# LeeBY68/Hier-SLAM

Hardware: AMD Instinct MI355X
Metric: fwd+bwd renders/sec @1200x680, 500k Gaussians, 4-level tree; grad max-abs-err vs ref (higher is better)
Workload: dtype f32; 1 GPU; semantic fwd+bwd render, 1200x680, P=500000 slam Gaussians, K=26 semantic channels, dense upstream grads on colour/semantic/depth/median/opacity; P=500000, visible=480888, num_rendered=1136056, width=1200, height=680, K=26, parallelism=single GPU, keyframes_per_rank=1

## Files before the change

### hier-slam_amd/csrc/hsr_sort.hip

```cpp
#include "hsr_common.h"

namespace {

constexpr int SORT_THREADS = 256;
constexpr int SORT_ITEMS = 16;
constexpr int SORT_TILE = SORT_THREADS * SORT_ITEMS;
static_assert(SORT_TILE == HSR_SORT_TILE, "hsr_common.h sizes the histogram scratch");

__global__ void __launch_bounds__(SORT_THREADS) sort_hist_kernel(const uint64_t* __restrict__ keys, int n, int shift,
                                                                 uint32_t mask, int nblocks, uint32_t* __restrict__ hist)
{
    __shared__ uint32_t h[256];
    h[threadIdx.x] = 0;
    __syncthreads();
    const int base = blockIdx.x * SORT_TILE;
#pragma unroll 4
    for (int i = 0; i < SORT_ITEMS; i++) {
        const int j = base + i * SORT_THREADS + threadIdx.x;
        if (j < n) atomicAdd(&h[(uint32_t)(keys[j] >> shift) & mask], 1u);
    }
    __syncthreads();
    hist[(size_t)threadIdx.x * nblocks + blockIdx.x] = h[threadIdx.x];
}

__global__ void __launch_bounds__(64) sort_rowscan_kernel(uint32_t* __restrict__ hist, int nblocks,
                                                           uint32_t* __restrict__ totals)
{
    const int lane = threadIdx.x;
    uint32_t* row = hist + (size_t)blockIdx.x * nblocks;
    uint32_t carry = 0;
    for (int base = 0; base < nblocks; base += 64) {
        const int j = base + lane;
        const uint32_t v = j < nblocks ? row[j] : 0u;
        uint32_t inc = v;
#pragma unroll
        for (int o = 1; o < 64; o <<= 1) {
            const uint32_t t = __shfl_up(inc, o);
            if (lane >= o) inc += t;
        }
        if (j < nblocks) row[j] = carry + inc - v;
        carry += __shfl(inc, 63);
    }
    if (lane == 0) totals[blockIdx.x] = carry;
}

__global__ void __launch_bounds__(SORT_THREADS) sort_scatter_kernel(const uint64_t* __restrict__ kin,
                                                                    const uint32_t* __restrict__ vin,
                                                                    uint64_t* __restrict__ kout, uint32_t* __restrict__ vout,
                                                                    int n, int shift, uint32_t mask, int nblocks,
                                                                    const uint32_t* __restrict__ hist_scanned,
                                                                    const uint32_t* __restrict__ totals)
{
    __shared__ uint32_t wcnt[4][256];
    __shared__ uint32_t dig_base[256];
    __shared__ uint32_t wtot[4];
    const int lane = threadIdx.x & 63, w = threadIdx.x >> 6;
#pragma unroll
    for (int i = 0; i < 4; i++) wcnt[i][threadIdx.x] = 0;
    __syncthreads();

    const int base = blockIdx.x * SORT_TILE + w * (64 * SORT_ITEMS);
    uint64_t key[SORT_ITEMS];
    uint32_t val[SORT_ITEMS];
    uint32_t rank[SORT_ITEMS];
    const uint64_t lt_mask = (1ull << lane) - 1ull;
    volatile uint32_t* mycnt = wcnt[w];
#pragma unroll
    for (int r = 0; r < SORT_ITEMS; r++) {
        const int j = base + r * 64 + lane;
        const bool valid = j < n;
        key[r] = valid ? kin[j] : 0ull;
        val[r] = valid ? vin[j] : 0u;
    }
#pragma unroll
    for (int r = 0; r < SORT_ITEMS; r++) {
        const int j = base + r * 64 + lane;
        const bool valid = j < n;
        const uint32_t d = (uint32_t)(key[r] >> shift) & mask;
        uint64_t m = __ballot(valid);
#pragma unroll
        for (int b = 0; b < 8; b++) {
            const bool bit = (d >> b) & 1u;
            const uint64_t bal = __ballot(bit);
            m &= bit ? bal : ~bal;
        }
        const uint32_t before = __popcll(m & lt_mask);
        const uint32_t prior = valid ? mycnt[d] : 0u;
        __builtin_amdgcn_wave_barrier();
        if (valid && before == 0) mycnt[d] = prior + (uint32_t)__popcll(m);
        __builtin_amdgcn_wave_barrier();
        rank[r] = prior + before;
    }
    {
        const uint32_t tv = totals[threadIdx.x];
        uint32_t inc = tv;
#pragma unroll
        for (int o = 1; o < 64; o <<= 1) {
            const uint32_t t = __shfl_up(inc, o);
            if (lane >= o) inc += t;
        }
        if (lane == 63) wtot[w] = inc;
        __syncthreads();
        uint32_t woff = 0;
#pragma unroll
        for (int i = 0; i < 4; i++) woff += i < w ? wtot[i] : 0u;
        dig_base[threadIdx.x] = woff + inc - tv;
    }
    {
        const uint32_t c0 = wcnt[0][threadIdx.x], c1 = wcnt[1][threadIdx.x], c2 = wcnt[2][threadIdx.x];
        const uint32_t g = dig_base[threadIdx.x] + hist_scanned[(size_t)threadIdx.x * nblocks + blockIdx.x];
        wcnt[0][threadIdx.x] = g;
        wcnt[1][threadIdx.x] = g + c0;
        wcnt[2][threadIdx.x] = g + c0 + c1;
        wcnt[3][threadIdx.x] = g + c0 + c1 + c2;
    }
    __syncthreads();
#pragma unroll
    for (int r = 0; r < SORT_ITEMS; r++) {
        const int j = base + r * 64 + lane;
        if (j < n) {
            const uint32_t d = (uint32_t)(key[r] >> shift) & mask;
            const uint32_t pos = wcnt[w][d] + rank[r];
            kout[pos] = key[r];
            vout[pos] = val[r];
        }
    }
}

}


constexpr int TS_MAX = 2048;

__device__ __forceinline__ void ts_block_radix(uint64_t* ka, uint32_t* va, uint64_t* kb, uint32_t* vb, int r0, int n,
                                               uint32_t* hist , uint32_t (*wcnt)[256], int gid_passes)
{
    const int t = threadIdx.x, lane = t & 63, w = t >> 6;
    const uint64_t lt = (1ull << lane) - 1ull;
    const int npass = gid_passes + 4;
    for (int pass = 0; pass < npass; pass++) {
        const bool on_gid = pass < gid_passes;
        const int shift = 8 * (on_gid ? pass : pass - gid_passes);
        hist[t] = 0;
#pragma unroll
        for (int i = 0; i < 4; i++) wcnt[i][t] = 0;
        __syncthreads();
        for (int i = t; i < n; i += 256)
            atomicAdd(&hist[((on_gid ? va[r0 + i] : (uint32_t)ka[r0 + i]) >> shift) & 255u], 1u);
        __syncthreads();
        {
            const uint32_t v = hist[t];
            uint32_t inc = v;
#pragma unroll
            for (int o = 1; o < 64; o <<= 1) {
                const uint32_t x = __shfl_up(inc, o);
                if (lane >= o) inc += x;
            }
            __shared__ uint32_t wt[4];
            if (lane == 63) wt[w] = inc;
            __syncthreads();
            uint32_t off = 0;
#pragma unroll
            for (int i = 0; i < 4; i++) off += i < w ? wt[i] : 0u;
            hist[t] = off + inc - v;
        }
        __syncthreads();
        for (int c = 0; c < n; c += 256) {
            const int i = c + t;
            const bool valid = i < n;
            const uint64_t k = valid ? ka[r0 + i] : 0ull;
            const uint32_t v = valid ? va[r0 + i] : 0u;
            const uint32_t d = ((on_gid ? v : (uint32_t)k) >> shift) & 255u;
            uint64_t m = __ballot(valid);
#pragma unroll
            for (int b = 0; b < 8; b++) {
                const bool bit = (d >> b) & 1u;
                const uint64_t bal = __ballot(bit);
                m &= bit ? bal : ~bal;
            }
            const uint32_t before = __popcll(m & lt);
            if (valid && before == 0) wcnt[w][d] = (uint32_t)__popcll(m);
            __syncthreads();
            if (valid) {
                uint32_t pos = hist[d] + before;
#pragma unroll
                for (int i2 = 0; i2 < 4; i2++) pos += i2 < w ? wcnt[i2][d] : 0u;
                kb[r0 + pos] = k;
                vb[r0 + pos] = v;
            }
            __syncthreads();
            hist[t] += wcnt[0][t] + wcnt[1][t] + wcnt[2][t] + wcnt[3][t];
#pragma unroll
            for (int i2 = 0; i2 < 4; i2++) wcnt[i2][t] = 0;
            __syncthreads();
        }
        uint64_t* tk = ka; ka = kb; kb = tk;
        uint32_t* tv = va; va = vb; vb = tv;
        __threadfence_block();
    }
    if (npass & 1) {
        __syncthreads();
        for (int i = t; i < n; i += 256) {
            kb[r0 + i] = ka[r0 + i];
            vb[r0 + i] = va[r0 + i];
        }
    }
}

constexpr int TP_MAX = 1024;
constexpr int TQ_MAX = 2048;

template <int E, int NT>
__device__ __forceinline__ void net_bitonic(uint64_t (&x)[E], int tid, ulonglong2* buf)
{
    constexpr int N = NT * E;
#pragma unroll
    for (int k = 2; k <= N; k <<= 1) {
#pragma unroll
        for (int j = k >> 1; j > 0; j >>= 1) {
            if (j < E) {
#pragma unroll
                for (int r = 0; r < E; r++) {
                    if ((r & j) == 0) {
                        const bool up = k < E ? ((r & k) == 0) : (((E * tid) & k) == 0);
                        const uint64_t a = x[r], b = x[r + j];
                        const bool sw = (a > b) == up;
                        x[r] = sw ? b : a;
                        x[r + j] = sw ? a : b;
                    }
                }
            } else {
                const int m = j / E;
                const bool cross = m >= 64;
#pragma unroll
                for (int q = 0; q < E / 2; q++) buf[q * NT + tid] = make_ulonglong2(x[2 * q], x[2 * q + 1]);
                if (cross) {
                    __syncthreads();
                } else {
                    __builtin_amdgcn_fence(__ATOMIC_RELEASE, "wavefront");
                    __builtin_amdgcn_wave_barrier();
                    __builtin_amdgcn_fence(__ATOMIC_ACQUIRE, "wavefront");
                }
                const bool keep_min = ((tid & m) == 0) == (((E * tid) & k) == 0);
#pragma unroll
                for (int q = 0; q < E / 2; q++) {
                    const ulonglong2 y = buf[q * NT + (tid ^ m)];
                    const uint64_t a0 = x[2 * q], a1 = x[2 * q + 1];
                    x[2 * q] = keep_min ? (a0 < y.x ? a0 : y.x) : (a0 > y.x ? a0 : y.x);
                    x[2 * q + 1] = keep_min ? (a1 < y.y ? a1 : y.y) : (a1 > y.y ? a1 : y.y);
                }
                if (cross) {
                    __syncthreads();
                } else {
                    __builtin_amdgcn_fence(__ATOMIC_RELEASE, "wavefront");
                    __builtin_amdgcn_wave_barrier();
                    __builtin_amdgcn_fence(__ATOMIC_ACQUIRE, "wavefront");
                }
            }
        }
    }
}

__device__ __forceinline__ void block_sort_tile(int tile, const uint2* __restrict__ ranges, uint64_t* __restrict__ keys,
                                                uint32_t* __restrict__ vals, uint64_t* __restrict__ keys_alt,
                                                uint32_t* __restrict__ vals_alt, int gid_passes, int composite_in, uint64_t* comp,
                                                uint32_t* hist, uint32_t (*wcnt)[256])
{
    const uint2 rg = ranges[tile];
    const int r0 = (int)rg.x, n = (int)(rg.y - rg.x);
    const int t = threadIdx.x;
    const uint64_t my_tile_hi = (uint64_t)tile << 32;
    if (n <= 0) return;
    if (n == 1 || n > TS_MAX) {
        if (composite_in) {
            for (int i = t; i < n; i += 256) {
                const uint64_t c = keys[r0 + i];
                keys[r0 + i] = my_tile_hi | (c >> 32);
                vals[r0 + i] = (uint32_t)c;
            }
            __syncthreads();
        }
        if (n == 1) return;
    }
    if (n > TS_MAX) {
        ts_block_radix(keys, vals, keys_alt, vals_alt, r0, n, hist, wcnt, gid_passes);
        return;
    }
    if (composite_in) {
        static_assert(TQ_MAX == TS_MAX && TS_MAX * 8 >= 4 * 256 * 16, "exchange buffer = the LDS network's key array");
        uint64_t x[8];
#pragma unroll
        for (int r = 0; r < 8; r++) {
            const int e = 8 * t + r;
            x[r] = e < n ? keys[r0 + e] : ~0ull;
        }
        net_bitonic<8, 256>(x, t, reinterpret_cast<ulonglong2*>(comp));
#pragma unroll
        for (int r = 0; r < 8; r++) {
            const int e = 8 * t + r;
            if (e < n) {
                keys[r0 + e] = my_tile_hi | (x[r] >> 32);
                vals[r0 + e] = (uint32_t)x[r];
            }
        }
        return;
    }
    int N = 64;
    while (N < n) N <<= 1;
    const uint64_t tile_hi = keys[r0] & 0xFFFFFFFF00000000ull;
    for (int i = t; i < N; i += 256)
        comp[i] = i < n ? (((keys[r0 + i] & 0xFFFFFFFFull) << 32) | (uint64_t)vals[r0 + i]) : ~0ull;
    __syncthreads();
    bool cross = false;
    for (int k = 2; k <= N; k <<= 1) {
        for (int j = k >> 1; j > 0; j >>= 1) {
            if (j >= 128 || cross) __syncthreads();
            cross = j >= 128;
            for (int i = t; i < N / 2; i += 256) {
                const int lo = ((i & ~(j - 1)) << 1) | (i & (j - 1));
                const int hi = lo | j;
                const bool up = (lo & k) == 0;
                const uint64_t a = comp[lo], b = comp[hi];
                if ((a > b) == up) {
                    comp[lo] = b;
                    comp[hi] = a;
                }
            }
        }
    }
    __syncthreads();
    for (int i = t; i < n; i += 256) {
        const uint64_t c = comp[i];
        keys[r0 + i] = tile_hi | (c >> 32);
        vals[r0 + i] = (uint32_t)c;
    }
}

__global__ void __launch_bounds__(256) tile_sort_kernel(const uint2* __restrict__ ranges, uint64_t* __restrict__ keys,
                                                        uint32_t* __restrict__ vals, uint64_t* __restrict__ keys_alt,
                                                        uint32_t* __restrict__ vals_alt, int gid_passes, int composite_in, BinDevRef ref)
{
    if (ref.base) {
        BinState bs;
        if (!hsr_bin_resolve(ref, *ref.R_dev, &bs)) return;
        keys = bs.keys; vals = bs.vals; keys_alt = bs.keys_unsorted; vals_alt = bs.vals_unsorted;
    }
    __shared__ uint64_t comp[TS_MAX];
    __shared__ uint32_t hist[256];
    __shared__ uint32_t wcnt[4][256];
    if (composite_in == 2) {
        const uint2 rg = ranges[blockIdx.x];
        if (rg.y - rg.x <= (uint32_t)TP_MAX) return;
        composite_in = 1;
    }
    block_sort_tile((int)blockIdx.x, ranges, keys, vals, keys_alt, vals_alt, gid_passes, composite_in, comp, hist, wcnt);
}

template <int E>
__device__ __forceinline__ void pair_sort_tile(int r0, int n, int tid, uint64_t tile_hi, uint64_t* __restrict__ keys,
                                               uint32_t* __restrict__ vals, ulonglong2* buf)
{
    uint64_t x[E];
#pragma unroll
    for (int r = 0; r < E; r++) {
        const int e = E * tid + r;
        x[r] = e < n ? keys[r0 + e] : ~0ull;
    }
    net_bitonic<E, 128>(x, tid, buf);
#pragma unroll
    for (int r = 0; r < E; r++) {
        const int e = E * tid + r;
        if (e < n) {
            keys[r0 + e] = tile_hi | (x[r] >> 32);
            vals[r0 + e] = (uint32_t)x[r];
        }
    }
}

__global__ void __launch_bounds__(256, 7) tile_sort_pair_kernel(int T, const uint2* __restrict__ ranges, uint64_t* __restrict__ keys,
                                                             uint32_t* __restrict__ vals, uint64_t* __restrict__ keys_alt,
                                                             uint32_t* __restrict__ vals_alt, int gid_passes, int big_too, BinDevRef ref)
{
    constexpr int RAW_WG = TS_MAX * 8 + 256 * 4 + 4 * 256 * 4, RAW_PAIR = 2 * 4 * 128 * 16;
    constexpr int RAW = RAW_WG > RAW_PAIR ? RAW_WG : RAW_PAIR;
    __shared__ __attribute__((aligned(16))) unsigned char s_raw[RAW];
    __shared__ int s_big[2];
    if (ref.base) {
        BinState bs;
        if (!hsr_bin_resolve(ref, *ref.R_dev, &bs)) return;
        keys = bs.keys; vals = bs.vals; keys_alt = bs.keys_unsorted; vals_alt = bs.vals_unsorted;
    }
    const int pair = threadIdx.x >> 7, tid = threadIdx.x & 127;
    const int tile = blockIdx.x * 2 + pair;
    int n = 0, r0 = 0;
    if (tile < T) {
        const uint2 rg = ranges[tile];
        r0 = (int)rg.x;
        n = (int)(rg.y - rg.x);
    }
    if (tid == 0) s_big[pair] = n > TP_MAX;
    {
        ulonglong2* buf = reinterpret_cast<ulonglong2*>(s_raw) + pair * (4 * 128);
        const uint64_t tile_hi = (uint64_t)tile << 32;
        if (n > 0 && n <= 256) pair_sort_tile<2>(r0, n, tid, tile_hi, keys, vals, buf);
        else if (n > 256 && n <= 512) pair_sort_tile<4>(r0, n, tid, tile_hi, keys, vals, buf);
        else if (n > 512 && n <= TP_MAX) pair_sort_tile<8>(r0, n, tid, tile_hi, keys, vals, buf);
        else { __syncthreads(); __syncthreads(); }
    }
    if (!big_too) return;
    __syncthreads();
    uint64_t* comp = reinterpret_cast<uint64_t*>(s_raw);
    uint32_t* hist = reinterpret_cast<uint32_t*>(s_raw + TS_MAX * 8);
    uint32_t (*wcnt)[256] = reinterpret_cast<uint32_t (*)[256]>(s_raw + TS_MAX * 8 + 256 * 4);
    for (int w = 0; w < 2; w++) {
        if (!s_big[w]) continue;
        block_sort_tile(blockIdx.x * 2 + w, ranges, keys, vals, keys_alt, vals_alt, gid_passes, 1, comp, hist, wcnt);
        __syncthreads();
    }
}

int hsr_sort_tile_passes(int end_bit)
{
    const int tile_bits = end_bit - 32;
    return tile_bits <= 0 ? 0 : (tile_bits + 7) / 8;
}
bool hsr_sort_emit_into_sorted_buffers(int end_bit) { return (hsr_sort_tile_passes(end_bit) & 1) == 0; }

int hsr_launch_sort_pairs(BinState& b, int R, int end_bit, int T, uint2* ranges, hipStream_t stream)
{
    if (R <= 0) return HSR_OK;
    const int passes = hsr_sort_tile_passes(end_bit);
    const int tile_bits = end_bit - 32;
    const int nblocks = (R + SORT_TILE - 1) / SORT_TILE;
    uint32_t* totals = b.hist + (size_t)256 * nblocks;
    uint64_t* ka = (passes & 1) ? b.keys_unsorted : b.keys;
    uint32_t* va = (passes & 1) ? b.vals_unsorted : b.vals;
    uint64_t* kb = (passes & 1) ? b.keys : b.keys_unsorted;
    uint32_t* vb = (passes & 1) ? b.vals : b.vals_unsorted;
    const int bits_per_pass = passes ? (tile_bits + passes - 1) / passes : 0;
    for (int p = 0; p < passes; p++) {
        const int shift = 32 + bits_per_pass * p;
        const int bits = min(bits_per_pass, end_bit - shift);
        const uint32_t mask = (1u << bits) - 1u;
        sort_hist_kernel<<<nblocks, SORT_THREADS, 0, stream>>>(ka, R, shift, mask, nblocks, b.hist);
        sort_rowscan_kernel<<<256, 64, 0, stream>>>(b.hist, nblocks, totals);
        sort_scatter_kernel<<<nblocks, SORT_THREADS, 0, stream>>>(ka, va, kb, vb, R, shift, mask, nblocks, b.hist, totals);
        uint64_t* tk = ka; ka = kb; kb = tk;
        uint32_t* tv = va; va = vb; vb = tv;
    }
    hsr_launch_tile_ranges_only(R, b.keys, ranges, stream);
    tile_sort_kernel<<<T, 256, 0, stream>>>(ranges, b.keys, b.vals, b.keys_unsorted, b.vals_unsorted, 0, 0, BinDevRef{nullptr, nullptr, 0});
    return HSR_OK;
}

int hsr_launch_tile_sort(BinState& b, int T, int P, const uint2* ranges, hipStream_t stream, const BinDevRef* ref, int avg_per_tile_hint)
{
    int bits = 0;
    while (bits < 32 && (1ull << bits) < (unsigned long long)(P > 1 ? P : 1)) bits++;
    const BinDevRef r = ref ? *ref : BinDevRef{nullptr, nullptr, 0};
    const bool many_big = avg_per_tile_hint > 800;
    tile_sort_pair_kernel<<<(T + 1) / 2, 256, 0, stream>>>(T, ranges, b.keys, b.vals, b.keys_unsorted, b.vals_unsorted, (bits + 7) / 8,
                                                           many_big ? 0 : 1, r);
    if (many_big)
        tile_sort_kernel<<<T, 256, 0, stream>>>(ranges, b.keys, b.vals, b.keys_unsorted, b.vals_unsorted, (bits + 7) / 8, 2, r);
    return HSR_OK;
}
```

Before: 1883 renders/s.

## Use ds_swizzle/permlane exchanges in bitonic tile sort and vectorize global I/O

The per-tile bitonic network now exchanges partners inside a wavefront using ds_swizzle and permlane32_swap register shuffles instead of writing to and reading back from LDS with wave barriers. Loads and stores of keys and values use 16-byte vector accesses when the segment is aligned. Pointers are also marked as global address space so the compiler can emit global rather than flat instructions. This is meant to cut LDS traffic and memory-instruction count in the tile sort stage, at the cost of two 32-bit shuffles per 64-bit element and more code complexity.

```diff
diff --git a/hier-slam_amd/csrc/hsr_sort.hip b/hier-slam_amd/csrc/hsr_sort.hip
--- a/hier-slam_amd/csrc/hsr_sort.hip
+++ b/hier-slam_amd/csrc/hsr_sort.hip
@@ -1,4 +1,5 @@
 #include "hsr_common.h"
+#include "hsr_sort_net.h"
 
 namespace {
 
@@ -132,7 +133,7 @@
 
 constexpr int TS_MAX = 2048;
 
-__device__ __forceinline__ void ts_block_radix(uint64_t* ka, uint32_t* va, uint64_t* kb, uint32_t* vb, int r0, int n,
+__device__ __forceinline__ void ts_block_radix(sg_u64* ka, sg_u32* va, sg_u64* kb, sg_u32* vb, int r0, int n,
                                                uint32_t* hist , uint32_t (*wcnt)[256], int gid_passes)
 {
     const int t = threadIdx.x, lane = t & 63, w = t >> 6;
@@ -194,8 +195,8 @@
             for (int i2 = 0; i2 < 4; i2++) wcnt[i2][t] = 0;
             __syncthreads();
         }
-        uint64_t* tk = ka; ka = kb; kb = tk;
-        uint32_t* tv = va; va = vb; vb = tv;
+        sg_u64* tk = ka; ka = kb; kb = tk;
+        sg_u32* tv = va; va = vb; vb = tv;
         __threadfence_block();
     }
     if (npass & 1) {
@@ -209,64 +210,14 @@
 
 constexpr int TP_MAX = 1024;
 constexpr int TQ_MAX = 2048;
-
-template <int E, int NT>
-__device__ __forceinline__ void net_bitonic(uint64_t (&x)[E], int tid, ulonglong2* buf)
-{
-    constexpr int N = NT * E;
-#pragma unroll
-    for (int k = 2; k <= N; k <<= 1) {
-#pragma unroll
-        for (int j = k >> 1; j > 0; j >>= 1) {
-            if (j < E) {
-#pragma unroll
-                for (int r = 0; r < E; r++) {
-                    if ((r & j) == 0) {
-                        const bool up = k < E ? ((r & k) == 0) : (((E * tid) & k) == 0);
-                        const uint64_t a = x[r], b = x[r + j];
-                        const bool sw = (a > b) == up;
-                        x[r] = sw ? b : a;
-                        x[r + j] = sw ? a : b;
-                    }
-                }
-            } else {
-                const int m = j / E;
-                const bool cross = m >= 64;
-#pragma unroll
-                for (int q = 0; q < E / 2; q++) buf[q * NT + tid] = make_ulonglong2(x[2 * q], x[2 * q + 1]);
-                if (cross) {
-                    __syncthreads();
-                } else {
-                    __builtin_amdgcn_fence(__ATOMIC_RELEASE, "wavefront");
-                    __builtin_amdgcn_wave_barrier();
-                    __builtin_amdgcn_fence(__ATOMIC_ACQUIRE, "wavefront");
-                }
-                const bool keep_min = ((tid & m) == 0) == (((E * tid) & k) == 0);
-#pragma unroll
-                for (int q = 0; q < E / 2; q++) {
-                    const ulonglong2 y = buf[q * NT + (tid ^ m)];
-                    const uint64_t a0 = x[2 * q], a1 = x[2 * q + 1];
-                    x[2 * q] = keep_min ? (a0 < y.x ? a0 : y.x) : (a0 > y.x ? a0 : y.x);
-                    x[2 * q + 1] = keep_min ? (a1 < y.y ? a1 : y.y) : (a1 > y.y ? a1 : y.y);
-                }
-                if (cross) {
-                    __syncthreads();
-                } else {
-                    __builtin_amdgcn_fence(__ATOMIC_RELEASE, "wavefront");
-                    __builtin_amdgcn_wave_barrier();
-                    __builtin_amdgcn_fence(__ATOMIC_ACQUIRE, "wavefront");
-                }
-            }
-        }
-    }
-}
-
-__device__ __forceinline__ void block_sort_tile(int tile, const uint2* __restrict__ ranges, uint64_t* __restrict__ keys,
-                                                uint32_t* __restrict__ vals, uint64_t* __restrict__ keys_alt,
-                                                uint32_t* __restrict__ vals_alt, int gid_passes, int composite_in, uint64_t* comp,
+constexpr int TS_XCH = SN_SWIZZLE;
+
+__device__ __forceinline__ void block_sort_tile(int tile, const sg_u32x2* __restrict__ ranges, sg_u64* __restrict__ keys,
+                                                sg_u32* __restrict__ vals, sg_u64* __restrict__ keys_alt,
+                                                sg_u32* __restrict__ vals_alt, int gid_passes, int composite_in, uint64_t* comp,
                                                 uint32_t* hist, uint32_t (*wcnt)[256])
 {
-    const uint2 rg = ranges[tile];
+    const sn_u32x2 rg = ranges[tile];
     const int r0 = (int)rg.x, n = (int)(rg.y - rg.x);
     const int t = threadIdx.x;
     const uint64_t my_tile_hi = (uint64_t)tile << 32;
@@ -288,21 +239,12 @@
     }
     if (composite_in) {
         static_assert(TQ_MAX == TS_MAX && TS_MAX * 8 >= 4 * 256 * 16, "exchange buffer = the LDS network's key array");
+        int tq = t;
+        asm volatile("" : "+v"(tq));
         uint64_t x[8];
-#pragma unroll
-        for (int r = 0; r < 8; r++) {
-            const int e = 8 * t + r;
-            x[r] = e < n ? keys[r0 + e] : ~0ull;
-        }
-        net_bitonic<8, 256>(x, t, reinterpret_cast<ulonglong2*>(comp));
-#pragma unroll
-        for (int r = 0; r < 8; r++) {
-            const int e = 8 * t + r;
-            if (e < n) {
-                keys[r0 + e] = my_tile_hi | (x[r] >> 32);
-                vals[r0 + e] = (uint32_t)x[r];
-            }
-        }
+        sn_load_run<8>(keys + r0, (r0 & 1) == 0, 8 * tq, n, x);
+        net_bitonic<8, 256, TS_XCH>(x, tq, reinterpret_cast<ulonglong2*>(comp));
+        sn_store_run<8>(keys + r0, vals + r0, r0, 8 * tq, n, my_tile_hi, x);
         return;
     }
     int N = 64;
@@ -345,36 +287,27 @@
         if (!hsr_bin_resolve(ref, *ref.R_dev, &bs)) return;
         keys = bs.keys; vals = bs.vals; keys_alt = bs.keys_unsorted; vals_alt = bs.vals_unsorted;
     }
+    const sg_u32x2* const ranges_g = (const sg_u32x2*)ranges;
     __shared__ uint64_t comp[TS_MAX];
     __shared__ uint32_t hist[256];
     __shared__ uint32_t wcnt[4][256];
     if (composite_in == 2) {
-        const uint2 rg = ranges[blockIdx.x];
+        const sn_u32x2 rg = ranges_g[blockIdx.x];
         if (rg.y - rg.x <= (uint32_t)TP_MAX) return;
         composite_in = 1;
     }
-    block_sort_tile((int)blockIdx.x, ranges, keys, vals, keys_alt, vals_alt, gid_passes, composite_in, comp, hist, wcnt);
+    block_sort_tile((int)blockIdx.x, ranges_g, (sg_u64*)keys, (sg_u32*)vals, (sg_u64*)keys_alt, (sg_u32*)vals_alt, gid_passes, composite_in,
+                    comp, hist, wcnt);
 }
 
 template <int E>
-__device__ __forceinline__ void pair_sort_tile(int r0, int n, int tid, uint64_t tile_hi, uint64_t* __restrict__ keys,
-                                               uint32_t* __restrict__ vals, ulonglong2* buf)
+__device__ __forceinline__ void pair_sort_tile(int r0, int n, int tid, uint64_t tile_hi, sg_u64* __restrict__ keys,
+                                               sg_u32* __restrict__ vals, ulonglong2* buf)
 {
     uint64_t x[E];
-#pragma unroll
-    for (int r = 0; r < E; r++) {
-        const int e = E * tid + r;
-        x[r] = e < n ? keys[r0 + e] : ~0ull;
-    }
-    net_bitonic<E, 128>(x, tid, buf);
-#pragma unroll
-    for (int r = 0; r < E; r++) {
-        const int e = E * tid + r;
-        if (e < n) {
-            keys[r0 + e] = tile_hi | (x[r] >> 32);
-            vals[r0 + e] = (uint32_t)x[r];
-        }
-    }
+    sn_load_run<E>(keys + r0, (r0 & 1) == 0, E * tid, n, x);
+    net_bitonic<E, 128, TS_XCH>(x, tid, buf);
+    sn_store_run<E>(keys + r0, vals + r0, r0, E * tid, n, tile_hi, x);
 }
 
 __global__ void __launch_bounds__(256, 7) tile_sort_pair_kernel(int T, const uint2* __restrict__ ranges, uint64_t* __restrict__ keys,
@@ -390,11 +323,14 @@
         if (!hsr_bin_resolve(ref, *ref.R_dev, &bs)) return;
         keys = bs.keys; vals = bs.vals; keys_alt = bs.keys_unsorted; vals_alt = bs.vals_unsorted;
     }
+    const sg_u32x2* const ranges_g = (const sg_u32x2*)ranges;
+    sg_u64* const keys_g = (sg_u64*)keys;
+    sg_u32* const vals_g = (sg_u32*)vals;
     const int pair = threadIdx.x >> 7, tid = threadIdx.x & 127;
     const int tile = blockIdx.x * 2 + pair;
     int n = 0, r0 = 0;
     if (tile < T) {
-        const uint2 rg = ranges[tile];
+        const sn_u32x2 rg = ranges_g[tile];
         r0 = (int)rg.x;
         n = (int)(rg.y - rg.x);
     }
@@ -402,9 +338,9 @@
     {
         ulonglong2* buf = reinterpret_cast<ulonglong2*>(s_raw) + pair * (4 * 128);
         const uint64_t tile_hi = (uint64_t)tile << 32;
-        if (n > 0 && n <= 256) pair_sort_tile<2>(r0, n, tid, tile_hi, keys, vals, buf);
-        else if (n > 256 && n <= 512) pair_sort_tile<4>(r0, n, tid, tile_hi, keys, vals, buf);
-        else if (n > 512 && n <= TP_MAX) pair_sort_tile<8>(r0, n, tid, tile_hi, keys, vals, buf);
+        if (n > 0 && n <= 256) pair_sort_tile<2>(r0, n, tid, tile_hi, keys_g, vals_g, buf);
+        else if (n > 256 && n <= 512) pair_sort_tile<4>(r0, n, tid, tile_hi, keys_g, vals_g, buf);
+        else if (n > 512 && n <= TP_MAX) pair_sort_tile<8>(r0, n, tid, tile_hi, keys_g, vals_g, buf);
         else { __syncthreads(); __syncthreads(); }
     }
     if (!big_too) return;
@@ -414,7 +350,7 @@
     uint32_t (*wcnt)[256] = reinterpret_cast<uint32_t (*)[256]>(s_raw + TS_MAX * 8 + 256 * 4);
     for (int w = 0; w < 2; w++) {
         if (!s_big[w]) continue;
-        block_sort_tile(blockIdx.x * 2 + w, ranges, keys, vals, keys_alt, vals_alt, gid_passes, 1, comp, hist, wcnt);
+        block_sort_tile(blockIdx.x * 2 + w, ranges_g, keys_g, vals_g, (sg_u64*)keys_alt, (sg_u32*)vals_alt, gid_passes, 1, comp, hist, wcnt);
         __syncthreads();
     }
 }
diff --git a/hier-slam_amd/csrc/hsr_sort_net.h b/hier-slam_amd/csrc/hsr_sort_net.h
--- /dev/null
+++ b/hier-slam_amd/csrc/hsr_sort_net.h
@@ -0,0 +1,185 @@
+#pragma once
+#include <hip/hip_runtime.h>
+#include <stdint.h>
+
+typedef __attribute__((address_space(1))) uint64_t sg_u64;
+typedef __attribute__((address_space(1))) uint32_t sg_u32;
+typedef uint64_t sn_u64x2 __attribute__((ext_vector_type(2)));
+typedef uint32_t sn_u32x2 __attribute__((ext_vector_type(2)));
+typedef uint32_t sn_u32x4 __attribute__((ext_vector_type(4)));
+typedef __attribute__((address_space(1))) sn_u64x2 sg_u64x2;
+typedef __attribute__((address_space(1))) sn_u32x2 sg_u32x2;
+typedef __attribute__((address_space(1))) sn_u32x4 sg_u32x4;
+
+enum { SN_LDS = 0, SN_BPERMUTE = 1, SN_SWIZZLE = 2, SN_DPP = 3, SN_MIX = 4 };
+
+template <int CTRL>
+__device__ __forceinline__ uint32_t sn_dpp(uint32_t v)
+{
+    return (uint32_t)__builtin_amdgcn_update_dpp(0, (int)v, CTRL, 0xf, 0xf, true);
+}
+
+template <int M>
+__device__ __forceinline__ uint32_t sn_swizzle_xor(uint32_t v)
+{
+    return (uint32_t)__builtin_amdgcn_ds_swizzle((int)v, 0x1f | (M << 10));
+}
+
+template <int XCH>
+__device__ __forceinline__ uint32_t sn_partner_dword(uint32_t v, int m, int lane)
+{
+    if (XCH == SN_BPERMUTE) return (uint32_t)__shfl_xor((int)v, m);
+    constexpr int QP_1032 = 0xB1, QP_2301 = 0x4E, QP_3210 = 0x1B, ROW_MIRROR = 0x140, ROW_HALF_MIRROR = 0x141;
+    if (XCH == SN_DPP || XCH == SN_MIX) {
+        switch (m) {
+        case 1: return sn_dpp<QP_1032>(v);
+        case 2: return sn_dpp<QP_2301>(v);
+        default: break;
+        }
+    }
+    if (XCH == SN_DPP) {
+        switch (m) {
+        case 4: return sn_dpp<QP_3210>(sn_dpp<ROW_HALF_MIRROR>(v));
+        case 8: return sn_dpp<ROW_HALF_MIRROR>(sn_dpp<ROW_MIRROR>(v));
+        case 16: {
+            const auto r = __builtin_amdgcn_permlane16_swap(v, v, false, false);
+            return (lane & 16) ? r[0] : r[1];
+        }
+        default: break;
+        }
+    }
+    switch (m) {
+    case 1: return sn_swizzle_xor<1>(v);
+    case 2: return sn_swizzle_xor<2>(v);
+    case 4: return sn_swizzle_xor<4>(v);
+    case 8: return sn_swizzle_xor<8>(v);
+    case 16: return sn_swizzle_xor<16>(v);
+    default: {
+        const auto r = __builtin_amdgcn_permlane32_swap(v, v, false, false);
+        return lane < 32 ? r[1] : r[0];
+    }
+    }
+}
+
+template <int E, int NT, int XCH = SN_LDS>
+__device__ __forceinline__ void net_bitonic(uint64_t (&x)[E], int tid, ulonglong2* buf)
+{
+    constexpr int N = NT * E;
+#pragma unroll
+    for (int k = 2; k <= N; k <<= 1) {
+#pragma unroll
+        for (int j = k >> 1; j > 0; j >>= 1) {
+            if (j < E) {
+#pragma unroll
+                for (int r = 0; r < E; r++) {
+                    if ((r & j) == 0) {
+                        const bool up = k < E ? ((r & k) == 0) : (((E * tid) & k) == 0);
+                        const uint64_t a = x[r], b = x[r + j];
+                        const bool sw = (a > b) == up;
+                        x[r] = sw ? b : a;
+                        x[r + j] = sw ? a : b;
+                    }
+                }
+            } else {
+                const int m = j / E;
+                const bool cross = m >= 64;
+                const bool keep_min = ((tid & m) == 0) == (((E * tid) & k) == 0);
+                if (cross || XCH == SN_LDS) {
+#pragma unroll
+                    for (int q = 0; q < E / 2; q++) buf[q * NT + tid] = make_ulonglong2(x[2 * q], x[2 * q + 1]);
+                    if (cross) {
+                        __syncthreads();
+                    } else {
+                        __builtin_amdgcn_fence(__ATOMIC_RELEASE, "wavefront");
+                        __builtin_amdgcn_wave_barrier();
+                        __builtin_amdgcn_fence(__ATOMIC_ACQUIRE, "wavefront");
+                    }
+#pragma unroll
+                    for (int q = 0; q < E / 2; q++) {
+                        const ulonglong2 y = buf[q * NT + (tid ^ m)];
+                        const uint64_t a0 = x[2 * q], a1 = x[2 * q + 1];
+                        x[2 * q] = ((a0 < y.x) == keep_min) ? a0 : y.x;
+                        x[2 * q + 1] = ((a1 < y.y) == keep_min) ? a1 : y.y;
+                    }
+                    if (cross) {
+                        __syncthreads();
+                    } else {
+                        __builtin_amdgcn_fence(__ATOMIC_RELEASE, "wavefront");
+                        __builtin_amdgcn_wave_barrier();
+                        __builtin_amdgcn_fence(__ATOMIC_ACQUIRE, "wavefront");
+                    }
+                } else {
+#pragma unroll
+                    for (int r = 0; r < E; r++) {
+                        const uint64_t a = x[r];
+                        const uint32_t ylo = sn_partner_dword<XCH>((uint32_t)a, m, tid & 63);
+                        const uint32_t yhi = sn_partner_dword<XCH>((uint32_t)(a >> 32), m, tid & 63);
+                        const uint64_t y = ((uint64_t)yhi << 32) | ylo;
+                        x[r] = ((a < y) == keep_min) ? a : y;
+                    }
+                }
+            }
+        }
+    }
+}
+
+template <int E>
+__device__ __forceinline__ void sn_load_run(const sg_u64* seg, bool seg_even, int e0, int n, uint64_t (&x)[E])
+{
+    if (seg_even && e0 + E <= n) {
+        const sg_u64x2* p = reinterpret_cast<const sg_u64x2*>(seg + e0);
+#pragma unroll
+        for (int q = 0; q < E / 2; q++) {
+            const sn_u64x2 v = p[q];
+            x[2 * q] = v.x;
+            x[2 * q + 1] = v.y;
+        }
+    } else {
+#pragma unroll
+        for (int r = 0; r < E; r++) x[r] = e0 + r < n ? seg[e0 + r] : ~0ull;
+    }
+}
+
+template <int E>
+__device__ __forceinline__ void sn_store_run(sg_u64* kseg, sg_u32* vseg, int r0, int e0, int n, uint64_t tile_hi, const uint64_t (&x)[E])
+{
+    const bool whole = e0 + E <= n;
+    if (whole && (r0 & 1) == 0) {
+        sg_u64x2* p = reinterpret_cast<sg_u64x2*>(kseg + e0);
+#pragma unroll
+        for (int q = 0; q < E / 2; q++) {
+            sn_u64x2 v;
+            v.x = tile_hi | (x[2 * q] >> 32);
+            v.y = tile_hi | (x[2 * q + 1] >> 32);
+            p[q] = v;
+        }
+    } else {
+#pragma unroll
+        for (int r = 0; r < E; r++)
+            if (e0 + r < n) kseg[e0 + r] = tile_hi | (x[r] >> 32);
+    }
+    constexpr int VA = E >= 4 ? 4 : 2;
+    if (whole && ((r0 + e0) & (VA - 1)) == 0) {
+        if constexpr (E >= 4) {
+            sg_u32x4* p = reinterpret_cast<sg_u32x4*>(vseg + e0);
+#pragma unroll
+            for (int q = 0; q < E / 4; q++) {
+                sn_u32x4 v;
+                v.x = (uint32_t)x[4 * q];
+                v.y = (uint32_t)x[4 * q + 1];
+                v.z = (uint32_t)x[4 * q + 2];
+                v.w = (uint32_t)x[4 * q + 3];
+                p[q] = v;
+            }
+        } else {
+            sn_u32x2 v;
+            v.x = (uint32_t)x[0];
+            v.y = (uint32_t)x[1];
+            *reinterpret_cast<sg_u32x2*>(vseg + e0) = v;
+        }
+    } else {
+#pragma unroll
+        for (int r = 0; r < E; r++)
+            if (e0 + r < n) vseg[e0 + r] = (uint32_t)x[r];
+    }
+}
```

Result: faster. 1906 renders/s, median of 6 (+1.3%).
